# nhcha6/embodied-object-detection

Measured on AMD Instinct MI355X. Metric: frames/sec (640x640, implicit_memory); frames/sec/GPU = value / n_gpus, higher is better.
Workload: dtype f32

## Files before the change

embodied_object_detection_amd/_lib.py:

```python
from __future__ import annotations

import ctypes as C
import os

HERE = os.path.dirname(os.path.abspath(__file__))
LIB_PATH = os.environ.get("EOD_LIB_PATH") or os.path.join(HERE, "libeod_hip.so")

c_f32p = C.c_void_p
c_i32p = C.c_void_p
c_void_p = C.c_void_p


class EodError(RuntimeError):
    pass


_ERR = {-1: "EOD_ERR_BAD_DIMS", -2: "EOD_ERR_ALIGN", -3: "EOD_ERR_LAUNCH", -4: "EOD_ERR_NULL", -5: "EOD_ERR_CAPACITY"}


MAX_BATCH = 8
MAX_LEVELS = 40
SEMMAP_SCORES = 0x10000
SEMMAP_LOCATE = 0x40000
SEMMAP_PEAKS = 0x80000
SEMMAP_K_SHIFT, SEMMAP_RADIUS_SHIFT, SEMMAP_Q_SHIFT = 12, 20, 24


class EodConvDesc(C.Structure):
    _fields_ = [
        ("x", C.c_void_p), ("w", C.c_void_p), ("bias", C.c_void_p), ("res", C.c_void_p), ("y", C.c_void_p),
        ("workspace", C.c_void_p), ("workspace_bytes", C.c_size_t), ("m_count", C.c_void_p), ("m_unit", C.c_int32),
        ("m_segments", C.c_int32),
        ("N", C.c_int32), ("H", C.c_int32), ("W", C.c_int32), ("Cin", C.c_int32), ("OH", C.c_int32), ("OW", C.c_int32),
        ("Cout", C.c_int32), ("KH", C.c_int32), ("KW", C.c_int32), ("stride", C.c_int32), ("pad", C.c_int32),
        ("Kpad", C.c_int32), ("relu", C.c_int32), ("res_mode", C.c_int32), ("in_relu", C.c_int32),
        ("out_mode", C.c_int32), ("tap4", C.c_int32), ("force_tile", C.c_int32), ("force_splitk", C.c_int32),
        ("out_scale", C.c_float), ("levels", C.c_int32), ("level_off", C.c_int32 * (MAX_LEVELS + 1)), ("level_h", C.c_int32 * MAX_LEVELS),
        ("level_w", C.c_int32 * MAX_LEVELS), ("fuse_w", C.c_void_p), ("out_units", C.c_void_p), ("fuse_b", C.c_float), ("w_split", C.c_void_p),
        ("plan_rows", C.c_int32), ("lds_reserve", C.c_int32), ("gn_partial", C.c_void_p), ("gn_groups", C.c_int32),
        ("y2", C.c_void_p), ("split_n", C.c_int32), ("prefetch2", C.c_int32), ("gate", C.c_void_p),
        ("w_half", C.c_void_p), ("math", C.c_int32),
    ]


class EodConvPlan(C.Structure):
    _fields_ = [(n, C.c_int32) for n in ("tile", "bm", "bn", "bk", "splitk", "cps", "nchunks", "wavek", "glds", "tiles_m", "tiles_n",
                                         "gn_fused")]


class EodBoxRefine(C.Structure):
    _fields_ = [("deltas", C.c_void_p), ("ld", C.c_int32), ("wx", C.c_float), ("wy", C.c_float), ("ww", C.c_float), ("wh", C.c_float),
                ("clip", C.c_int32), ("img_w", C.c_float), ("img_h", C.c_float), ("boxes_out", C.c_void_p)]


class EodCenterNetLossDesc(C.Structure):
    _fields_ = [
        ("head_out", C.c_void_p), ("head_stride", C.c_int32), ("P", C.c_int32), ("levels", C.c_int32), ("level_off", C.c_int32 * 9),
        ("level_scale", C.c_float * 8), ("agn_heatmap", C.c_void_p), ("reg_targets", C.c_void_p), ("pos_inds", C.c_void_p),
        ("n_pos", C.c_int32), ("hm_focal_alpha", C.c_float), ("hm_focal_beta", C.c_float), ("loss_gamma", C.c_float),
        ("sigmoid_clamp", C.c_float), ("ignore_high_fp", C.c_float), ("pos_weight", C.c_float), ("neg_weight", C.c_float),
        ("reg_weight", C.c_float), ("num_pos_avg", C.c_float), ("reg_norm", C.c_float), ("counts_local", C.c_void_p),
        ("counts_total", C.c_void_p), ("world_size", C.c_float), ("d_head_out", C.c_void_p),
        ("losses", C.c_void_p), ("workspace", C.c_void_p), ("workspace_bytes", C.c_size_t),
    ]


class EodCenterNetTargetDesc(C.Structure):
    _fields_ = [
        ("gt_boxes", C.c_void_p), ("n_boxes", C.c_int32), ("levels", C.c_int32), ("level_off", C.c_int32 * 9), ("level_w", C.c_int32 * 8),
        ("level_stride", C.c_int32 * 8), ("soi_lo", C.c_float * 8), ("soi_hi", C.c_float * 8), ("hm_min_overlap", C.c_double),
        ("min_radius", C.c_double), ("agn_heatmap", C.c_void_p), ("reg_targets", C.c_void_p), ("pos_inds", C.c_void_p),
        ("counts", C.c_void_p),
    ]


class EodProposalDesc(C.Structure):
    _fields_ = [
        ("head_out", C.c_void_p), ("head_stride", C.c_int32), ("levels", C.c_int32), ("level_off", C.c_int32 * 6),
        ("level_w", C.c_int32 * 5), ("level_stride", C.c_int32 * 5), ("level_scale", C.c_float * 5),
        ("score_thresh", C.c_float), ("pre_nms_topk", C.c_int32), ("post_nms_topk", C.c_int32), ("nms_thresh", C.c_float),
# ... 152 lines not shown
    "eod_place_masks_workspace_bytes": (C.c_size_t, [C.c_int, C.c_int]),
    "eod_place_masks": (C.c_int, [C.c_void_p] * 4 + [C.c_int] * 7 + [C.c_void_p, C.c_void_p, C.c_size_t, C.c_void_p]),
}

REGIONS_SIGNATURES = {
    "eod_map_regions_workspace_bytes": (C.c_size_t, [C.c_int] * 3),
    "eod_map_regions": (C.c_int, [C.c_void_p] + [C.c_int] * 3 + [C.c_float] + [C.c_int] * 3 + [C.c_void_p] * 3 + [C.c_size_t, C.c_void_p]),
}

INVENTORY_SIGNATURES = {
    "eod_map_inventory_workspace_bytes": (C.c_size_t, [C.c_int] * 4),
    "eod_map_inventory": (C.c_int, [C.c_void_p] * 3 + [C.c_int] * 4 + [C.c_float] + [C.c_int] * 3 + [C.c_void_p] * 3 + [C.c_size_t, C.c_void_p]),
}

DESCRIBE_SIGNATURES = {
    "eod_describe_pool": (C.c_int, [C.c_void_p] * 3 + [C.c_int] * 2 + [C.c_void_p] * 5),
    "eod_describe_classify": (C.c_int, [C.c_void_p] * 2 + [C.c_int] * 3 + [C.c_void_p] * 4),
}

RELATIONS_SIGNATURES = {
    "eod_map_relations": (C.c_int, [C.c_void_p] * 2 + [C.c_int] * 6 + [C.c_void_p] * 12),
}

ROUTE_SIGNATURES = {
    "eod_map_route_workspace_bytes": (C.c_size_t, [C.c_int] * 2),
    "eod_map_route": (C.c_int, [C.c_void_p] * 3 + [C.c_int] * 8 + [C.c_void_p] * 11 + [C.c_size_t, C.c_void_p]),
}

CLEARANCE_SIGNATURES = {
    "eod_map_clearance_workspace_bytes": (C.c_size_t, [C.c_int] * 2),
    "eod_map_clearance": (C.c_int, [C.c_void_p] * 3 + [C.c_int] * 6 + [C.c_void_p] * 13 + [C.c_size_t, C.c_void_p]),
}

_lib = None


def load():
    global _lib
    if _lib is not None:
        return _lib
    if not os.path.exists(LIB_PATH):
        raise EodError(
            f"{LIB_PATH} is missing: the HIP extension is not built. Run `python -m embodied_object_detection_amd.build` "
            "(hipcc --offload-arch=gfx950). There is no CPU fallback for the product path.")
    lib = C.CDLL(LIB_PATH)
    for name, (res, args) in {**SIGNATURES, **PLACE_SIGNATURES, **REGIONS_SIGNATURES, **INVENTORY_SIGNATURES,
                              **DESCRIBE_SIGNATURES, **RELATIONS_SIGNATURES, **ROUTE_SIGNATURES, **CLEARANCE_SIGNATURES}.items():
        fn = getattr(lib, name)
        fn.restype = res
        fn.argtypes = args
    _lib = lib
    return lib


def check(status: int, what: str):
    if status != 0:
        raise EodError(f"{what} failed: {_ERR.get(status, status)}")
```

embodied_object_detection_amd/build.py:

```python
from __future__ import annotations

import os
import subprocess
import sys

HERE = os.path.dirname(os.path.abspath(__file__))
CSRC = os.path.join(HERE, "csrc")
LIB = os.path.join(HERE, "libeod_hip.so")
SOURCES = ["conv_igemm.hip", "conv_fp32.hip", "conv_pointwise.hip", "conv_bf16x3.hip", "conv_f16.hip", "elementwise.hip", "roi_align.hip", "select.hip", "heads.hip", "memory.hip", "semmap.hip", "place.hip", "regions.hip", "inventory.hip", "memory_read.hip", "memory_backward.hip", "conv_wgrad.hip", "train_losses.hip", "describe.hip", "relations.hip", "route.hip", "clearance.hip"]
ARCH = "gfx950"


def _stale() -> bool:
    if not os.path.exists(LIB):
        return True
    t = os.path.getmtime(LIB)
    deps = [os.path.join(CSRC, f) for f in os.listdir(CSRC)] + [os.path.join(HERE, "..", "include", h) for h in ("eod_hip.h", "eod_place.h", "eod_regions.h", "eod_inventory.h", "eod_describe.h", "eod_relations.h", "eod_route.h", "eod_clearance.h")]
    return any(os.path.getmtime(d) > t for d in deps if os.path.exists(d))


def _usage_file(src: str) -> str:
    return os.path.join(HERE, "build", src.replace(".hip", ".usage.txt"))


def resource_usage() -> dict:
    import re
    out = {}
    for src in SOURCES:
        f = _usage_file(src)
        if not os.path.exists(f):
            continue
        cur = None
        for line in open(f):
            m = re.search(r"Function Name: (\S+)", line)
            if m:
                cur = out.setdefault(m.group(1), {})
                continue
            for key, pat in (("vgprs", r"\bVGPRs: (\d+)"), ("scratch", r"ScratchSize \[bytes/lane\]: (\d+)"),
                             ("occupancy", r"Occupancy \[waves/SIMD\]: (\d+)"), ("lds", r"LDS Size \[bytes/block\]: (\d+)")):
                m = re.search(pat, line)
                if m and cur is not None:
                    cur[key] = int(m.group(1))
    return out


def scratch_offenders(usage: dict = None) -> list:
    usage = resource_usage() if usage is None else usage
    return sorted(k for k, v in usage.items() if v.get("scratch", 0) > 0)


# ... 50 lines not shown
```

embodied_object_detection_amd/csrc/conv_common.h:

```cpp
#pragma once
#include "eod_common.h"
#include "conv_border_order.h"
#include "../../include/eod_hip.h"

namespace eodconv {


struct ConvArgs {
  const float* x;
  const float* w;
  const float* bias;
  const float* res;
  const float* gate;
  float* y;
  float* partial;
  const int* m_count;
  int m_unit;
  int m_segs, seg_rows;
  const float* fuse_w;
  const int* out_units;
  float fuse_b;
  int N, H, W, Cin, OH, OW, Cout, KH, KW, stride, pad, Kpad;
  int M, nchunks, splitk, cps;
  int relu, res_mode, in_relu, out_mode;
  int tiles_m, tiles_n;
  float out_scale;
  int nlv;
  int lv_off[EOD_MAX_LEVELS + 1], lv_h[EOD_MAX_LEVELS], lv_w[EOD_MAX_LEVELS];
  unsigned x_bytes, w_bytes;
  const void* w3;
  unsigned w3_bytes;
  const void* wh;
  unsigned wh_bytes;
  double* gn_partial;
  int gn_groups;
  float* y2;
  int split_n;
  FastDiv div_ow, div_oh, div_cd, div_row;
  int border;
  FastDiv div_bh, div_bw, div_bi;
};

__device__ __forceinline__ int conv_row_limit(const ConvArgs& p, int M) {
  if (p.m_count && p.m_segs <= 1) {
    const int lim = *p.m_count * p.m_unit;
    M = lim < M ? lim : M;
  }
  return M;
}

__device__ __forceinline__ bool conv_row_active(const ConvArgs& p, int m) {
  if (!p.m_count || p.m_segs <= 1) return true;
  const int s = m / p.seg_rows;
  return m - s * p.seg_rows < p.m_count[s] * p.m_unit;
}

__device__ __forceinline__ bool conv_tile_active(const ConvArgs& p, int m0, int bm) {
  if (!p.m_count || p.m_segs <= 1) return true;
  const int last = (m0 + bm - 1 < p.M ? m0 + bm - 1 : p.M - 1);
  const int s0 = m0 / p.seg_rows, s1 = last / p.seg_rows;
  if (m0 - s0 * p.seg_rows < p.m_count[s0] * p.m_unit) return true;
  for (int s = s0 + 1; s <= s1; ++s)
    if (p.m_count[s] > 0) return true;
  return false;
}

__device__ __forceinline__ int border_rois(const ConvArgs& p) {
  const int c = *p.m_count;
  return c < p.N ? c : p.N;
}
__device__ __forceinline__ int border_storage_row(const ConvArgs& p, int m, int rois) {
  const BorderRow b = border_row(m, rois, p.OH, p.OW, p.div_ow, p.div_bh, p.div_bw, p.div_bi);
  return (b.img * p.OH + b.oy) * p.OW + b.ox;
// ... 98 lines not shown
```

embodied_object_detection_amd/csrc/conv_fp32.hip:

```cpp
#include "conv_operands.h"

namespace eodconv {
namespace {

template <int BM, int BN, int BK, bool TAP4, bool MULTI, int PIPE = 0>
__global__ __launch_bounds__(256) void conv_igemm_kernel(ConvArgs p) {
  constexpr bool BORDER = PIPE == 3;
  static_assert(!BORDER || (BM == 64 && BN == 64 && BK == 32 && !TAP4 && !MULTI), "border-major order: the plain 64x64 kernel");
  constexpr bool PF2 = PIPE == 1;
  constexpr bool DB = PIPE == 2;
  constexpr int LS = BK + 4;
  constexpr int TM = BM / 64, TN = BN / 64;
  constexpr int QPR = BK / 4;
  constexpr int RPP = 256 / QPR;
  constexpr int AR = BM / RPP, BR = BN / RPP;
  static_assert(!TAP4 || BK == 32, "the stem path stages one 7x7 tap per float4: BK must be 32");
  constexpr int BUF = (BM + BN) * LS;
  __shared__ __attribute__((aligned(16))) float lds[(DB ? 2 : 1) * BUF];
  float* As = lds;
  float* Bs = lds + BM * LS;

  const int tid = threadIdx.x;
  const int lane = tid & 63;
  const int wave = tid >> 6;
  const int wm = wave >> 1, wn = wave & 1;

  int M, tile_m, tile_n;
  if constexpr (BORDER) {
    if (!conv_claim_tile_border<BM>(p, M, tile_m, tile_n)) return;
  } else {
    const int t = conv_first_tile<BM>(p, M);
    if (t < 0) return;
    tile_m = t / p.tiles_n;
    tile_n = t - tile_m * p.tiles_n;
  }
  const int m0 = tile_m * BM, n0 = tile_n * BN;
  if (!conv_tile_active(p, m0, BM)) return;
  const int z = blockIdx.y;
  int c_end;
  const int c_begin = conv_chunk_range(p, p.cps, z, c_end);

  const int lr = tid / QPR, lq = tid % QPR;
  int a_off[AR], a_iy[AR], a_ix[AR];
  unsigned a_voff[AR];
  unsigned long long a_mask[AR];
  unsigned a_pitch[MULTI ? AR : 1];
  const int rois = BORDER ? border_rois(p) : 0;
#pragma unroll
  for (int i = 0; i < AR; ++i) {
    const int m = m0 + lr + RPP * i;
    const bool rowok = m < M;
    RowOrigin o;
    if constexpr (BORDER) o = conv_row_origin_border(p, m, rowok, rois);
    else o = conv_row_origin<MULTI>(p, m, rowok);
    a_iy[i] = rowok ? o.iy0 : -(1 << 28);
    a_ix[i] = o.ix0;
    a_off[i] = o.off;
    if (!TAP4) conv_row_address<MULTI>(p, o, rowok, lq, a_voff[i], a_mask[i], a_pitch[MULTI ? i : 0]);
  }
  unsigned w_voff[BR];
#pragma unroll
  for (int j = 0; j < BR; ++j) w_voff[j] = conv_w_row_offset(p, n0 + lr + RPP * j, lq);
  const __amdgpu_buffer_rsrc_t rsrc_x = conv_buffer(p.x, p.x_bytes);
  const __amdgpu_buffer_rsrc_t rsrc_w = conv_buffer(p.w, p.w_bytes);

  unsigned live = 0;
  if constexpr (BORDER) {
// ... 182 lines not shown
      if (tid < BM) {
        const int wr = tid >> 5, rr = tid & 31;
        const float v = red[(wr * 2 + 0) * 32 + rr] + red[(wr * 2 + 1) * 32 + rr] + p.fuse_b;
        const int m = m0 + tid;
        if (m < M) {
          const int tq = (int)fdiv((unsigned)m, p.div_ow);
          const int ox = m - tq * p.OW;
          const int img = (int)fdiv((unsigned)tq, p.div_oh);
          const int oy = tq - img * p.OH;
          const int unit = p.out_units ? p.out_units[img] : img;
          const int dy = tile_n >> 1, dx = tile_n & 1;
          p.y[((size_t)unit * 2 * p.OH + 2 * oy + dy) * (2 * p.OW) + 2 * ox + dx] = eod_sigmoid_precise(v);
        }
      }
      return;
    }
  }
  store_wave_tiles<TM, TN, BM == 64 && BN == 64, BORDER>(p, acc, m0 + wm * TM * 32, n0 + wn * TN * 32, M, z, lane);
}


template <int NW, bool MULTI>
__global__ __launch_bounds__(NW * 64) void conv_wavek_kernel(ConvArgs p) {
  constexpr int BK = 32;
  constexpr int LS = BK + 4;
  constexpr int AR = 4;
  __shared__ __attribute__((aligned(16))) float lds[NW * 2 * 32 * LS];
  const int tid = threadIdx.x;
  const int lane = tid & 63;
  const int wave = tid >> 6;
  float* As = lds + wave * (2 * 32 * LS);
  float* Bs = As + 32 * LS;

  int M;
  const int t = conv_first_tile<32>(p, M);
  if (t < 0) return;
  const int tile_m = t / p.tiles_n;
  const int tile_n = t - tile_m * p.tiles_n;
  const int m0 = tile_m * 32, n0 = tile_n * 32;
  if (!conv_tile_active(p, m0, 32)) return;

  int c_end;
  const int c_begin = conv_chunk_range(p, (p.nchunks + NW - 1) / NW, wave, c_end);

  const int lr = lane >> 3, lq = lane & 7;
  unsigned a_voff[AR];
  unsigned long long a_mask[AR];
  unsigned a_pitch[MULTI ? AR : 1];
  unsigned w_voff[AR];
#pragma unroll
  for (int i = 0; i < AR; ++i) {
    conv_row_address<MULTI>(p, m0 + lr + 8 * i, M, lq, a_voff[i], a_mask[i], a_pitch[MULTI ? i : 0]);
    w_voff[i] = conv_w_row_offset(p, n0 + lr + 8 * i, lq);
  }
  const __amdgpu_buffer_rsrc_t rsrc_x = conv_buffer(p.x, p.x_bytes);
  const __amdgpu_buffer_rsrc_t rsrc_w = conv_buffer(p.w, p.w_bytes);

  f32x4 ar0[AR], br0[AR], ar1[AR], br1[AR];
  ChunkWalker<BK, MULTI> walk(p, c_begin);
  auto load_chunk = [&](int chunk, f32x4 (&ar)[AR], f32x4 (&br)[AR]) {
    const int k0 = chunk * BK;
    const TapInfo ti = walk.next(p);
#pragma unroll
    for (int i = 0; i < AR; ++i) ar[i] = conv_load_a<MULTI>(rsrc_x, ti, a_voff[i], a_mask[i], a_pitch[MULTI ? i : 0]);
    if (p.in_relu) {
#pragma unroll
      for (int i = 0; i < AR; ++i) ar[i] = conv_relu4(ar[i]);
    }
#pragma unroll
    for (int j = 0; j < AR; ++j)
      br[j] = __builtin_bit_cast(f32x4, __builtin_amdgcn_raw_buffer_load_b128(rsrc_w, w_voff[j], k0 * 4, 0));
// ... 112 lines not shown
```

embodied_object_detection_amd/csrc/conv_igemm.hip:

```cpp
#include "conv_common.h"
#include "../../include/eod_hip.h"
#include <atomic>
#include <cstdlib>
#include <cstring>

namespace {

using namespace eodconv;

template <int VEC>
__global__ __launch_bounds__(256) void conv_splitk_reduce_kernel(ConvArgs p) {
  EOD_CHAIN_PRIO();
  const int M = conv_row_limit(p, p.M);
  const unsigned per_row = (unsigned)p.Cout / VEC;
  const unsigned total = (unsigned)M * per_row;
  const size_t slab = (size_t)p.M * p.Cout;
  for (unsigned idx = blockIdx.x * blockDim.x + threadIdx.x; idx < total; idx += gridDim.x * blockDim.x) {
    const unsigned m = fdiv(idx, p.div_row);
    if (!conv_row_active(p, (int)m)) continue;
    const unsigned n = (idx - m * per_row) * VEC;
    const float* src = p.partial + (size_t)m * p.Cout + n;
    if (VEC == 4) {
      f32x4 v = {0.f, 0.f, 0.f, 0.f};
      for (int zb = 0; zb < p.splitk; zb += 4) {
        f32x4 t[4];
#pragma unroll
        for (int j = 0; j < 4; ++j)
          if (zb + j < p.splitk) t[j] = *reinterpret_cast<const f32x4*>(src + (size_t)(zb + j) * slab);
#pragma unroll
        for (int j = 0; j < 4; ++j)
          if (zb + j < p.splitk) v += t[j];
      }
      epilogue_store<true>(p, v.x, (int)m, (int)n);
      epilogue_store<true>(p, v.y, (int)m, (int)n + 1);
// ... 57 lines not shown
    red[sub][col / cpg4][0] = s;
    red[sub][col / cpg4][1] = q;
  }
  __syncthreads();
  if ((int)threadIdx.x < p.gn_groups) {
    double ts = 0.0, tq = 0.0;
    for (int u = 0; u < nsub; ++u) {
      ts += red[u][threadIdx.x][0];
      tq += red[u][threadIdx.x][1];
    }
    p.gn_partial[((size_t)blockIdx.x * p.gn_groups + threadIdx.x) * 2 + 0] = ts;
    p.gn_partial[((size_t)blockIdx.x * p.gn_groups + threadIdx.x) * 2 + 1] = tq;
  }
}

std::atomic<int>& math_mode() {
  static std::atomic<int> v([] {
    const char* e = getenv("EOD_CONV_MATH");
    if (e && strcmp(e, "bf16x3") == 0) return EOD_MATH_BF16X3;
    if (e && strcmp(e, "f16") == 0) return EOD_MATH_F16;
    return EOD_MATH_FP32;
  }());
  return v;
}

struct Plan {
  int tile;
  int bk;
  int glds;
  int bm, bn, tiles_m, tiles_n, splitk, cps, nchunks;
  int wavek;
  int pw_np;
  int border;
};

constexpr int kForcePointwise = 30;

int effective_math(const EodConvDesc* d) { return d->math > 0 ? d->math - 1 : math_mode().load(std::memory_order_relaxed); }

bool pointwise_eligible(const EodConvDesc* d) {
  return effective_math(d) == EOD_MATH_FP32 && d->KH == 1 && d->KW == 1 && d->stride == 1 && d->pad == 0 && d->levels <= 0 && !d->tap4 &&
         d->Cin == d->Kpad && (d->Cin == 64 || d->Cin == 128 || d->Cin == 256) && d->Cout % 64 == 0 && d->out_mode == 0 &&
         (d->res_mode == 0 || d->res_mode == 1) && !d->in_relu && !d->gate && !d->m_count && d->split_n == 0 && !d->gn_partial &&
         d->lds_reserve == 0;
}

constexpr int kForceBorder = 43;
constexpr bool kBorderAuto = true;

bool border_eligible(const EodConvDesc* d) {
  return effective_math(d) == EOD_MATH_FP32 && d->KH == 3 && d->KW == 3 && d->stride == 1 && d->pad == 1 && d->levels <= 0 && !d->tap4 &&
         d->m_count && d->m_segments <= 1 && d->m_unit == d->OH * d->OW && d->OH >= 3 && d->OW >= 3 && d->Cin % 32 == 0 &&
         d->out_mode == 0 && d->res_mode == 0 && !d->in_relu && !d->gate && d->split_n == 0 && !d->gn_partial && d->prefetch2 == 0;
}

Plan make_plan(const EodConvDesc* d, int M) {
  static const int cfg[5][2] = {{128, 128}, {128, 64}, {64, 64}, {256, 128}, {64, 256}};
  Plan pl{};
  int pick = 2;
  const int ft = d->force_tile % 10, fbk = d->force_tile / 10;
  const bool half_ok = !d->tap4 && !d->in_relu;
  const bool f16_forced = (fbk == 8 || fbk == 9) && half_ok;
  if (f16_forced) pick = ft == 4 ? 3 : 2;
  else if (ft >= 1 && ft <= 3) pick = ft - 1;
  else if (ft == 4 && fbk == 5 && half_ok) pick = 3;
  const bool bk64_ok = !d->tap4 && d->Cin % 64 == 0 && d->Kpad % 64 == 0;
  pl.glds = f16_forced ? 3 : ((fbk == 5 && half_ok) ? 2 : 0);
// ... 67 lines not shown
  const bool pw_auto = d->force_tile == 0 && d->force_splitk == 0 && pointwise_eligible(d) && pl.splitk == 1 && !pl.wavek && tiles >= 256 &&
                       !(d->Kpad == 256 && d->Cout < 1024);
  if (pw_forced || pw_auto) {
    const int panels = d->Cout / 64;
    const long row_tiles = (Mp + 63) / 64;
    const long want = tiles >= 256 ? 512 : 1;
    int np = 1;
    for (int cand = 4; cand > 1; cand >>= 1)
      if (panels >= cand && row_tiles * ((panels + cand - 1) / cand) >= want) {
        np = cand;
        break;
      }
    pl.pw_np = np;
    pl.tile = 6;
    pl.glds = 0;
    pl.bk = 32;
    pl.nchunks = d->Kpad / 32;
    pl.bm = 64;
    pl.bn = 64 * np;
    pl.tiles_m = (M + 63) / 64;
    pl.tiles_n = (panels + np - 1) / np;
    pl.splitk = 1;
    pl.cps = pl.nchunks;
    pl.wavek = 0;
  }
  const bool border_forced = d->force_tile == kForceBorder && d->force_splitk <= 1;
  const bool border_auto = kBorderAuto && d->force_tile == 0 && border_eligible(d) && pl.glds == 0 && pl.tile == 3 && pl.bk == 32 &&
                           pl.splitk == 1 && !pl.wavek;
  if (border_forced) {
    pl.splitk = 1;
    pl.cps = pl.nchunks;
  }
  pl.border = (border_forced || border_auto) ? 1 : 0;
  return pl;
}

int total_rows(const EodConvDesc* d) { return d->levels > 0 ? d->level_off[d->levels] : d->N * d->OH * d->OW; }

int check_desc(const EodConvDesc* d) {
  if (!d || !d->x || !d->w || !d->y) return EOD_ERR_NULL;
  if (d->N <= 0 || d->Cin <= 0 || d->Cout <= 0) return EOD_ERR_BAD_DIMS;
  if (d->levels <= 0 && (d->H <= 0 || d->W <= 0 || d->OH <= 0 || d->OW <= 0)) return EOD_ERR_BAD_DIMS;
  if (d->KH <= 0 || d->KW <= 0 || d->stride <= 0 || d->pad < 0) return EOD_ERR_BAD_DIMS;
  if (d->Kpad % 32 != 0 || d->Kpad < d->KH * d->KW * d->Cin) return EOD_ERR_BAD_DIMS;
  if (d->tap4) {
    if (d->Cin != 4) return EOD_ERR_BAD_DIMS;
  } else {
    if (d->Cin % 32 != 0 || d->Kpad != d->KH * d->KW * d->Cin) return EOD_ERR_BAD_DIMS;
  }
  if (d->levels > 0) {
    if (d->levels > EOD_MAX_LEVELS || d->N != 1 || d->stride != 1 || d->KH != d->KW || d->pad != d->KH / 2 || d->tap4 || d->out_mode != 0 ||
        d->res_mode == 2 || d->level_off[0] != 0)
      return EOD_ERR_BAD_DIMS;
    for (int l = 0; l < d->levels; ++l)
      if (d->level_h[l] <= 0 || d->level_w[l] <= 0 || d->level_off[l + 1] - d->level_off[l] != d->level_h[l] * d->level_w[l])
        return EOD_ERR_BAD_DIMS;
  } else {
    if (d->OH != (d->H + 2 * d->pad - d->KH) / d->stride + 1) return EOD_ERR_BAD_DIMS;
    if (d->OW != (d->W + 2 * d->pad - d->KW) / d->stride + 1) return EOD_ERR_BAD_DIMS;
  }
  if (d->levels <= 0 && (long)d->N * d->H * d->W * d->Cin >= (1L << 29)) return EOD_ERR_BAD_DIMS;
  if ((long)d->Cout * d->Kpad >= (1L << 29)) return EOD_ERR_BAD_DIMS;
  if (d->KH * d->KW > 64) return EOD_ERR_BAD_DIMS;
  if ((long)total_rows(d) * (d->Cout > d->Cin ? d->Cout : d->Cin) >= (1L << 31)) return EOD_ERR_BAD_DIMS;
  if (d->out_mode == 1 && (d->Cout % 4 != 0)) return EOD_ERR_BAD_DIMS;
  if (d->out_mode == 2) {
// ... 17 lines not shown
  if (d->gate && (d->force_tile / 10 == 8 || d->force_tile / 10 == 9) &&
      (d->math != EOD_MATH_F16 + 1 || d->force_tile % 10 != 3 || d->levels > 0 || d->tap4 || d->in_relu))
    return EOD_ERR_BAD_DIMS;
  if (d->math < 0 || d->math > EOD_MATH_F16 + 1) return EOD_ERR_BAD_DIMS;
  if ((d->force_tile / 10 == 8 || d->force_tile / 10 == 9) && d->force_tile % 10 != 3 && d->force_tile % 10 != 4) return EOD_ERR_BAD_DIMS;
  if (d->lds_reserve < 0 || d->lds_reserve > 48 * 1024) return EOD_ERR_BAD_DIMS;
  if (d->force_tile == kForcePointwise && (!pointwise_eligible(d) || d->force_splitk > 1)) return EOD_ERR_BAD_DIMS;
  if (d->force_tile == kForceBorder && (!border_eligible(d) || d->force_splitk > 1)) return EOD_ERR_BAD_DIMS;
  if (d->split_n != 0) {
    if (!d->y2) return EOD_ERR_NULL;
    if (d->split_n < 0 || d->split_n >= d->Cout || d->out_mode != 0 || d->res_mode != 0 || d->levels > 0 || d->gn_partial)
      return EOD_ERR_BAD_DIMS;
  }
  if (d->gn_partial) {
    const int cpg = d->gn_groups > 0 ? d->Cout / d->gn_groups : 0;
    if (d->levels <= 0 || d->m_count || d->out_mode != 0 || d->gn_groups <= 0 || d->gn_groups > 64 || d->Cout % d->gn_groups != 0 ||
        cpg > 64 || (cpg & (cpg - 1)) != 0 || cpg < 4 || d->Cout % 4 != 0 || d->Cout > 1024 || 256 % (d->Cout / 4) != 0 ||
        64 % (cpg / 4) != 0)
      return EOD_ERR_BAD_DIMS;
  }
  if (!eod_aligned16(d->x) || !eod_aligned16(d->w) || !eod_aligned16(d->w_split) || !eod_aligned16(d->w_half)) return EOD_ERR_ALIGN;
  return EOD_OK;
}

}

extern "C" int eod_set_conv_math(int mode) {
  if (mode != EOD_MATH_FP32 && mode != EOD_MATH_BF16X3 && mode != EOD_MATH_F16) return EOD_ERR_BAD_DIMS;
  return math_mode().exchange(mode);
}

extern "C" int eod_get_conv_math(void) { return math_mode().load(); }

extern "C" size_t eod_conv_split_weights_bytes(int Cout, int Kpad) {
  return (Cout > 0 && Kpad > 0 && Kpad % 32 == 0) ? (size_t)Cout * Kpad * 6 : 0;
}

extern "C" int eod_conv_split_weights_bf16x3(const float* w, int Cout, int Kpad, void* out, eod_stream_t stream) {
  if (!w || !out) return EOD_ERR_NULL;
  if (Cout <= 0 || Kpad <= 0 || Kpad % 32 != 0 || (long)Cout * Kpad * 6 >= (1L << 32)) return EOD_ERR_BAD_DIMS;
  if (!eod_aligned16(w) || !eod_aligned16(out)) return EOD_ERR_ALIGN;
  launch_split_weights(w, out, Cout, Kpad, static_cast<hipStream_t>(stream));
  return eod_launch_status();
}

extern "C" size_t eod_conv_half_weights_bytes(int Cout, int Kpad) {
  return (Cout > 0 && Kpad > 0 && Kpad % 32 == 0) ? (size_t)Cout * Kpad * 2 : 0;
}

extern "C" int eod_conv_half_weights(const float* w, int Cout, int Kpad, void* out, eod_stream_t stream) {
  if (!w || !out) return EOD_ERR_NULL;
  if (Cout <= 0 || Kpad <= 0 || Kpad % 32 != 0 || (long)Cout * Kpad >= (1L << 29)) return EOD_ERR_BAD_DIMS;
  if (!eod_aligned16(w) || !eod_aligned16(out)) return EOD_ERR_ALIGN;
  launch_half_weights(w, out, Cout, Kpad, static_cast<hipStream_t>(stream));
  return eod_launch_status();
}

extern "C" int eod_conv2d_gn_fused(const EodConvDesc* d) {
  EodConvDesc t = *d;
  t.gn_partial = nullptr;
  if (check_desc(&t) != EOD_OK) return 0;
  return make_plan(&t, total_rows(&t)).splitk > 1 ? 1 : 0;
}

extern "C" int eod_conv2d_plan(const EodConvDesc* d, EodConvPlan* out) {
  if (!out) return EOD_ERR_NULL;
  const int st = check_desc(d);
  if (st != EOD_OK) return st;
  const Plan pl = make_plan(d, total_rows(d));
  out->tile = pl.tile; out->bm = pl.bm; out->bn = pl.bn; out->bk = pl.bk;
  out->splitk = pl.splitk; out->cps = pl.cps; out->nchunks = pl.nchunks;
  out->wavek = pl.wavek; out->glds = pl.glds;
  out->tiles_m = pl.tiles_m; out->tiles_n = pl.tiles_n;
  out->gn_fused = (d->gn_partial && pl.splitk > 1) ? 1 : 0;
  return EOD_OK;
}

extern "C" size_t eod_conv2d_workspace_bytes(const EodConvDesc* d) {
  if (check_desc(d) != EOD_OK) return 0;
  const int M = total_rows(d);
  const Plan pl = make_plan(d, M);
  if (pl.splitk <= 1) return 0;
  return (size_t)pl.splitk * M * d->Cout * sizeof(float);
}

extern "C" int eod_conv2d(const EodConvDesc* d, eod_stream_t stream) {
  const int st = check_desc(d);
  if (st != EOD_OK) return st;
  hipStream_t s = static_cast<hipStream_t>(stream);
  ConvArgs a{};
  a.x = d->x; a.w = d->w; a.bias = d->bias; a.res = d->res; a.y = d->y;
  a.partial = d->workspace;
  a.m_count = d->m_count; a.m_unit = d->m_unit;
  a.m_segs = d->m_segments > 1 ? d->m_segments : 1;
  a.seg_rows = a.m_segs > 1 ? (d->N / d->m_segments) * d->OH * d->OW : 0;
  a.fuse_w = d->fuse_w; a.out_units = d->out_units; a.fuse_b = d->fuse_b;
  a.N = d->N; a.H = d->H; a.W = d->W; a.Cin = d->Cin; a.OH = d->OH; a.OW = d->OW; a.Cout = d->Cout;
  a.KH = d->KH; a.KW = d->KW; a.stride = d->stride; a.pad = d->pad; a.Kpad = d->Kpad;
  a.M = total_rows(d);
  a.div_ow = eod_make_fastdiv((unsigned)(d->OW > 0 ? d->OW : 1));
  a.div_oh = eod_make_fastdiv((unsigned)(d->OH > 0 ? d->OH : 1));
  a.div_row = eod_make_fastdiv((unsigned)(d->Cout % 4 == 0 ? d->Cout / 4 : d->Cout));
  a.div_cd = eod_make_fastdiv((unsigned)((d->Cout >> 2) > 0 ? (d->Cout >> 2) : 1));
  a.div_bh = eod_make_fastdiv((unsigned)(d->OH > 2 ? d->OH - 2 : 1));
  a.div_bw = eod_make_fastdiv((unsigned)(d->OW > 2 ? d->OW - 2 : 1));
  a.div_bi = eod_make_fastdiv((unsigned)(d->OH > 2 && d->OW > 2 ? (d->OH - 2) * (d->OW - 2) : 1));
  {
    const size_t xe = d->levels > 0 ? (size_t)d->level_off[d->levels] * d->Cin : (size_t)d->N * d->H * d->W * d->Cin;
    a.x_bytes = (unsigned)(xe * sizeof(float));
    a.w_bytes = (unsigned)((size_t)d->Cout * d->Kpad * sizeof(float));
    a.w3 = d->w_split;
    a.w3_bytes = (unsigned)((size_t)d->Cout * d->Kpad * 6);
    a.wh = d->w_half;
    a.wh_bytes = (unsigned)((size_t)d->Cout * d->Kpad * 2);
  }
  a.nlv = d->levels > 0 ? d->levels : 0;
  for (int l = 0; l < a.nlv; ++l) {
    a.lv_off[l] = d->level_off[l];
    a.lv_h[l] = d->level_h[l];
    a.lv_w[l] = d->level_w[l];
  }
  if (a.nlv) a.lv_off[a.nlv] = d->level_off[a.nlv];
  a.relu = d->relu; a.res_mode = d->res_mode; a.in_relu = d->in_relu; a.out_mode = d->out_mode;
  a.gate = d->gate;
  a.out_scale = d->out_scale;
  a.gn_partial = d->gn_partial;
  a.gn_groups = d->gn_groups;
  a.y2 = d->y2;
  a.split_n = d->split_n;
  const Plan pl = make_plan(d, a.M);
  if (d->gn_partial && pl.splitk <= 1) return EOD_ERR_BAD_DIMS;
  a.nchunks = pl.nchunks;
  a.splitk = pl.splitk; a.cps = pl.cps; a.tiles_m = pl.tiles_m; a.tiles_n = pl.tiles_n;
  a.border = pl.border;
  if (pl.splitk > 1) {
    const size_t need = (size_t)pl.splitk * a.M * a.Cout * sizeof(float);
    if (!d->workspace || d->workspace_bytes < need) return EOD_ERR_CAPACITY;
  }
  dim3 grid(pl.tiles_m * pl.tiles_n, pl.splitk);
  if (pl.border) grid.x = (pl.tiles_m + 7) / 8 * 8 * pl.tiles_n;
  if (pl.pw_np) launch_conv_pointwise(a, pl.pw_np, grid, s);
  else if (pl.wavek) launch_conv_wavek(a, pl.wavek, grid, s);
  else if (pl.glds == 3) launch_conv_f16(a, pl.tile, pl.bk, grid, s);
  else if (pl.glds == 2) launch_conv_bf16x3(a, pl.tile, grid, s);
  else launch_conv_fp32(a, pl.tile, pl.bk, d->tap4 != 0, grid, s, d->lds_reserve, d->prefetch2);
  if (pl.splitk > 1) {
    const size_t total = (size_t)a.M * a.Cout;
    const bool vec = a.Cout % 4 == 0;
    int blocks = (int)((total / (vec ? 4 : 1) + 255) / 256);
    if (blocks > 2048) blocks = 2048;
    if (blocks < 1) blocks = 1;
    if (a.gn_partial) {
      int chunks = 0;
      for (int l = 0; l < a.nlv; ++l) chunks += (a.lv_off[l + 1] - a.lv_off[l] + EOD_GN_ROWS - 1) / EOD_GN_ROWS;
      hipLaunchKernelGGL(conv_splitk_reduce_gn_kernel, dim3(chunks), dim3(256), 0, s, a);
    } else if (vec) hipLaunchKernelGGL(conv_splitk_reduce_kernel<4>, dim3(blocks), dim3(256), 0, s, a);
    else hipLaunchKernelGGL(conv_splitk_reduce_kernel<1>, dim3(blocks), dim3(256), 0, s, a);
  }
  return eod_launch_status();
}
```

embodied_object_detection_amd/csrc/conv_operands.h:

```cpp
#pragma once
#include "conv_common.h"

namespace eodconv {

template <int BM>
__device__ __forceinline__ int conv_first_tile(const ConvArgs& p, int& M) {
  M = conv_row_limit(p, p.M);
  const int ntiles = ((M + BM - 1) / BM) * p.tiles_n;
  if ((int)blockIdx.x >= ntiles) return -1;
  return xcd_remap(blockIdx.x, ntiles);
}

template <int BM>
__device__ __forceinline__ bool conv_claim_tile_border(const ConvArgs& p, int& M, int& tile_m, int& tile_n) {
  M = conv_row_limit(p, p.M);
  const int live = (M + BM - 1) / BM;
  const int xcd = blockIdx.x & 7, k = blockIdx.x >> 3;
  const int g = k / p.tiles_n;
  const int r = g * 8 + xcd;
  tile_n = k - g * p.tiles_n;
  tile_m = live - 1 - r;
  return r < live;
}

__device__ __forceinline__ int conv_chunk_range(const ConvArgs& p, int per, int idx, int& c_end) {
  const int c_begin = idx * per;
  c_end = c_begin + per;
  if (c_end > p.nchunks) c_end = p.nchunks;
  return c_begin;
}

struct RowOrigin {
  int iy0, ix0, off, hh, ww;
};
template <bool MULTI>
__device__ __forceinline__ RowOrigin conv_row_origin(const ConvArgs& p, int m, bool rowok) {
  RowOrigin o = {0, 0, 0, 1, 1};
  if (rowok) {
    if (MULTI) {
      int l = 0;
      while (l + 1 < p.nlv && m >= p.lv_off[l + 1]) ++l;
      const int local = m - p.lv_off[l];
      o.ww = p.lv_w[l];
// ... 117 lines not shown
```

embodied_object_detection_amd/csrc/conv_pointwise.hip:

```cpp
#include "conv_operands.h"

namespace eodconv {
namespace {

template <int K>
struct PointwiseCfg {
  static constexpr int BKW = K == 256 ? 16 : 32;
  static constexpr int LSA = K + 4;
  static constexpr int LSW = BKW + 4;
  static constexpr int A_FLOATS = 64 * LSA;
  static constexpr int W_FLOATS = 64 * LSW;
  static constexpr int LDS_BYTES = (A_FLOATS + 2 * W_FLOATS) * 4;
  static constexpr int WG_PER_CU = K == 256 ? 2 : 3;
};

template <int K>
__global__ __launch_bounds__(256) __attribute__((amdgpu_waves_per_eu(PointwiseCfg<K>::WG_PER_CU))) void conv_pointwise_kernel(ConvArgs p, int np) {
  using Cfg = PointwiseCfg<K>;
  constexpr int BKW = Cfg::BKW, LSA = Cfg::LSA, LSW = Cfg::LSW;
  constexpr int NC = K / BKW;
  constexpr int KS = BKW / 8;
  constexpr int QPR = BKW / 4;
  constexpr int RPP = 256 / QPR;
  constexpr int BR = 64 / RPP;
  constexpr int AQ = K / 4;
  constexpr int AR = K / 16;
  static_assert(NC % 2 == 0, "stage parity");
  extern __shared__ __attribute__((aligned(16))) float lds[];
  float* As = lds;
  float* Ws = lds + Cfg::A_FLOATS;

  const int tid = threadIdx.x;
  const int lane = tid & 63;
  const int wave = tid >> 6;
  const int wm = wave >> 1, wn = wave & 1;

  int M;
  const int t = conv_first_tile<64>(p, M);
  if (t < 0) return;
  const int tile_m = t / p.tiles_n;
  const int grp = t - tile_m * p.tiles_n;
  const int m0 = tile_m * 64;
  const int panels = p.Cout >> 6;
  const int p0 = grp * np;
  const int p1 = p0 + np < panels ? p0 + np : panels;

  const __amdgpu_buffer_rsrc_t rsrc_x = conv_buffer(p.x, p.x_bytes);
  const __amdgpu_buffer_rsrc_t rsrc_w = conv_buffer(p.w, p.w_bytes);

  const int lr = tid / QPR, lq = tid % QPR;
  auto load_w = [&](int panel, int c, f32x4 (&wr)[BR]) {
    if (c >= NC) {
      c -= NC;
      ++panel;
    }
    if (panel >= p1) return;
#pragma unroll
    for (int j = 0; j < BR; ++j)
      wr[j] = __builtin_bit_cast(f32x4, __builtin_amdgcn_raw_buffer_load_b128(rsrc_w, conv_w_row_offset(p, panel * 64 + lr + RPP * j, lq),
                                                                              c * BKW * 4, 0));
  };
  auto store_w = [&](int buf, const f32x4 (&wr)[BR]) {
#pragma unroll
    for (int j = 0; j < BR; ++j) *reinterpret_cast<f32x4*>(Ws + buf * Cfg::W_FLOATS + (lr + RPP * j) * LSW + 4 * lq) = wr[j];
  };

  const int half = lane >> 5;
  const int m_base = m0 + wm * 32 + 4 * half;
  const int n_lane = wn * 32 + (lane & 31);
  auto load_res = [&](int panel, float (&rr)[16], float& bb) {
    const int n = panel * 64 + n_lane;
    if (p.bias) bb = p.bias[n];
    if (p.res_mode == 1) {
#pragma unroll
// ... 115 lines not shown
```

embodied_object_detection_amd/ops.py:

```python
from __future__ import annotations

import ctypes as C
from typing import Dict, Optional, Sequence, Tuple

import numpy as np
import torch

from . import _lib
from ._lib import EodConvDesc, EodDetDesc, EodMemWriteDesc, EodProposalDesc, check


_raw_stream = getattr(torch._C, "_cuda_getCurrentRawStream", None)


def _stream() -> int:
    if _raw_stream is not None:
        return _raw_stream(torch.cuda.current_device())
    return torch.cuda.current_stream().cuda_stream


def _ptr(t: Optional[torch.Tensor]) -> Optional[int]:
    return None if t is None else t.data_ptr()


# ... 8 lines not shown
    def __init__(self):
        self.bufs = {}

    def get(self, nbytes: int, device) -> torch.Tensor:
        key = (device.index if isinstance(device, torch.device) else str(device), _stream())
        buf = self.bufs.get(key)
        if buf is None or buf.numel() < nbytes:
            buf = torch.empty(max(int(nbytes), 1 << 20), dtype=torch.uint8, device=device)
            self.bufs[key] = buf
        return buf


_conv_ws = Workspace()


_CONV_MATH = {"fp32": 0, "bf16x3": 1, "f16": 2}
WGRAD_F16 = 512


def set_conv_math(mode: str) -> str:
    if mode not in _CONV_MATH:
        hint = ""
        if str(mode).lower() == "fp16":
            hint = (' ("fp16" / FP16 is the config key of autocast training: modeling.training.build_trainer / AmpTrainer, which choose '
                    'the arithmetic per launch; the process-wide inference arithmetic is "f16")')
        raise ValueError(f"conv math must be one of {sorted(_CONV_MATH)}, got {mode!r}{hint}")
    prev = _lib.load().eod_set_conv_math(_CONV_MATH[mode])
    check(min(prev, 0), "eod_set_conv_math")
    return {v: k for k, v in _CONV_MATH.items()}[prev]


def get_conv_math() -> str:
    return {v: k for k, v in _CONV_MATH.items()}[_lib.load().eod_get_conv_math()]


def fold_bn(w: torch.Tensor, bn_w, bn_b, bn_mean, bn_var, eps: float = 1e-5):
    scale = bn_w / torch.sqrt(bn_var + eps)
    return w * scale.view(-1, 1, 1, 1), bn_b - bn_mean * scale


def pack_conv_weight(w_oihw: torch.Tensor, cin_pad: Optional[int] = None) -> Tuple[torch.Tensor, int]:
    O, I, KH, KW = w_oihw.shape
    w = w_oihw.permute(0, 2, 3, 1).contiguous()
    if cin_pad is not None and cin_pad != I:
        wp = torch.zeros((O, KH, KW, cin_pad), dtype=w.dtype)
        wp[..., :I] = w
        w = wp
    K = w.shape[1] * w.shape[2] * w.shape[3]
    Kpad = (K + 31) // 32 * 32
    out = torch.zeros((O, Kpad), dtype=torch.float32)
    out[:, :K] = w.reshape(O, K)
    return out.contiguous(), Kpad


class Conv:

    def __init__(self, w_oihw: torch.Tensor, bias: Optional[torch.Tensor], stride: int = 1, pad: int = 0,
                 device="cuda", cin_pad: Optional[int] = None, deconv: bool = False, name: str = ""):
        self.name = name
        if deconv:
            Cin, Cout, kh, kw = w_oihw.shape
            assert kh == 2 and kw == 2
            w = w_oihw.permute(2, 3, 1, 0).reshape(4 * Cout, Cin, 1, 1).contiguous()
            self.out_mode = 1
            self.KH = self.KW = 1
            self.stride, self.pad = 1, 0
# ... 1644 lines not shown
```

include/eod_hip.h:

```cpp
#ifndef EOD_HIP_H
#define EOD_HIP_H
#include <stddef.h>
#include <stdint.h>

#ifdef __cplusplus
extern "C" {
#endif

typedef void* eod_stream_t;

#define EOD_OK 0
#define EOD_ERR_BAD_DIMS (-1)
#define EOD_ERR_ALIGN (-2)
#define EOD_ERR_LAUNCH (-3)
#define EOD_ERR_NULL (-4)
#define EOD_ERR_CAPACITY (-5)

#define EOD_MAX_BATCH 8
#define EOD_MAX_LEVELS 40

int eod_abi_version(void);

typedef struct EodConvDesc {
  const float* x;
// ... 15 lines not shown
  int32_t force_tile;
  int32_t force_splitk;
  float out_scale;
  int32_t levels;
  int32_t level_off[EOD_MAX_LEVELS + 1];
  int32_t level_h[EOD_MAX_LEVELS];
  int32_t level_w[EOD_MAX_LEVELS];
  const float* fuse_w;
  const int32_t* out_units;
  float fuse_b;
  const void* w_split;
  int32_t plan_rows;
  int32_t lds_reserve;
  double* gn_partial;
  int32_t gn_groups;
  float* y2;
  int32_t split_n;
  int32_t prefetch2;
  const float* gate;
  const void* w_half;
  int32_t math;
} EodConvDesc;
int eod_conv2d(const EodConvDesc* d, eod_stream_t stream);
int eod_conv2d_gn_fused(const EodConvDesc* d);
size_t eod_conv2d_workspace_bytes(const EodConvDesc* d);
typedef struct EodConvPlan {
  int32_t tile;
  int32_t bm, bn, bk;
  int32_t splitk, cps, nchunks;
  int32_t wavek;
  int32_t glds;
  int32_t tiles_m, tiles_n;
  int32_t gn_fused;
} EodConvPlan;
int eod_conv2d_plan(const EodConvDesc* d, EodConvPlan* out);
#define EOD_MATH_FP32 0
#define EOD_MATH_BF16X3 1
#define EOD_MATH_F16 2
int eod_set_conv_math(int mode);
int eod_get_conv_math(void);
size_t eod_conv_split_weights_bytes(int Cout, int Kpad);
int eod_conv_split_weights_bf16x3(const float* w, int Cout, int Kpad, void* out, eod_stream_t stream);
size_t eod_conv_half_weights_bytes(int Cout, int Kpad);
int eod_conv_half_weights(const float* w, int Cout, int Kpad, void* out, eod_stream_t stream);

int eod_preprocess_image(const uint8_t* img_chw, float* out_nhwc4, int H, int W, int Hp, int Wp,
                         const float* mean3, const float* std3, eod_stream_t stream);
int eod_maxpool3x3s2(const float* x, float* y, int N, int H, int W, int C, int OH, int OW, eod_stream_t stream);
size_t eod_groupnorm_workspace_bytes(const int32_t* level_off_host, int levels, int groups);
int eod_groupnorm_relu(const float* x, float* y, const float* gamma, const float* beta, const int32_t* level_off_host,
                       int levels, int C, int groups, float eps, float* stats, int partial_ready, eod_stream_t stream);
size_t eod_groupnorm_partial_offset(int levels, int groups);
size_t eod_groupnorm_backward_workspace_bytes(const int32_t* level_off_host, int levels, int C);
int eod_groupnorm_relu_backward(const float* x, const float* y, const float* dy, const float* gamma, const int32_t* level_off_host,
                                int levels, int C, int groups, float eps, const float* fwd_stats, void* workspace, float* dx,
                                float* dgamma, float* dbeta, eod_stream_t stream);
int eod_mask_predictor_sigmoid(const float* x, const float* w, float bias, float* prob, int rows, int C,
                               const int32_t* unit_count, int unit_rows, const int32_t* out_units ,
                               eod_stream_t stream);

typedef struct EodBoxRefine {
  const float* deltas;
  int32_t ld;
  float wx, wy, ww, wh;
  int32_t clip;
  float img_w, img_h;
// ... 294 lines not shown
```

Baseline: 322.9.

## Choose row- or column-major conv tile order per layer from an L2 fetch model

Adds a per-launch tile rasterization order for the implicit-GEMM conv kernels. A host-side model estimates how many A (activation) and B (weight) tile bytes each XCD's contiguous range of tiles would fetch under row-major versus column-major order, then picks the cheaper one. In auto mode this applies only to wavek==4 plans without glds, border or out_mode 2. The goal is less redundant operand traffic through each XCD's L2. Kernels now go through a shared conv_claim_tile helper, and the EodConvPlan struct gains a field, which changes the ABI.

Result: no change. 320.1 (-0.9%).

```diff
diff --git a/embodied_object_detection_amd/_lib.py b/embodied_object_detection_amd/_lib.py
--- a/embodied_object_detection_amd/_lib.py
+++ b/embodied_object_detection_amd/_lib.py
@@ -45,7 +45,7 @@
 
 class EodConvPlan(C.Structure):
     _fields_ = [(n, C.c_int32) for n in ("tile", "bm", "bn", "bk", "splitk", "cps", "nchunks", "wavek", "glds", "tiles_m", "tiles_n",
-                                         "gn_fused")]
+                                         "gn_fused", "order")]
 
 
 class EodBoxRefine(C.Structure):
@@ -264,6 +264,11 @@
     "eod_map_clearance": (C.c_int, [C.c_void_p] * 3 + [C.c_int] * 6 + [C.c_void_p] * 13 + [C.c_size_t, C.c_void_p]),
 }
 
+CONV_ORDER_SIGNATURES = {
+    "eod_set_conv_tile_order": (C.c_int, [C.c_int]),
+    "eod_get_conv_tile_order": (C.c_int, []),
+}
+
 _lib = None
 
 
@@ -277,7 +282,8 @@
             "(hipcc --offload-arch=gfx950). There is no CPU fallback for the product path.")
     lib = C.CDLL(LIB_PATH)
     for name, (res, args) in {**SIGNATURES, **PLACE_SIGNATURES, **REGIONS_SIGNATURES, **INVENTORY_SIGNATURES,
-                              **DESCRIBE_SIGNATURES, **RELATIONS_SIGNATURES, **ROUTE_SIGNATURES, **CLEARANCE_SIGNATURES}.items():
+                              **DESCRIBE_SIGNATURES, **RELATIONS_SIGNATURES, **ROUTE_SIGNATURES, **CLEARANCE_SIGNATURES,
+                              **CONV_ORDER_SIGNATURES}.items():
         fn = getattr(lib, name)
         fn.restype = res
         fn.argtypes = args
diff --git a/embodied_object_detection_amd/build.py b/embodied_object_detection_amd/build.py
--- a/embodied_object_detection_amd/build.py
+++ b/embodied_object_detection_amd/build.py
@@ -15,7 +15,7 @@
     if not os.path.exists(LIB):
         return True
     t = os.path.getmtime(LIB)
-    deps = [os.path.join(CSRC, f) for f in os.listdir(CSRC)] + [os.path.join(HERE, "..", "include", h) for h in ("eod_hip.h", "eod_place.h", "eod_regions.h", "eod_inventory.h", "eod_describe.h", "eod_relations.h", "eod_route.h", "eod_clearance.h")]
+    deps = [os.path.join(CSRC, f) for f in os.listdir(CSRC)] + [os.path.join(HERE, "..", "include", h) for h in ("eod_hip.h", "eod_place.h", "eod_regions.h", "eod_inventory.h", "eod_describe.h", "eod_relations.h", "eod_route.h", "eod_clearance.h", "eod_conv_order.h")]
     return any(os.path.getmtime(d) > t for d in deps if os.path.exists(d))
 
 
diff --git a/embodied_object_detection_amd/csrc/conv_common.h b/embodied_object_detection_amd/csrc/conv_common.h
--- a/embodied_object_detection_amd/csrc/conv_common.h
+++ b/embodied_object_detection_amd/csrc/conv_common.h
@@ -1,6 +1,7 @@
 #pragma once
 #include "eod_common.h"
 #include "conv_border_order.h"
+#include "conv_tile_order.h"
 #include "../../include/eod_hip.h"
 
 namespace eodconv {
@@ -39,6 +40,7 @@
   FastDiv div_ow, div_oh, div_cd, div_row;
   int border;
   FastDiv div_bh, div_bw, div_bi;
+  int order;
 };
 
 __device__ __forceinline__ int conv_row_limit(const ConvArgs& p, int M) {
diff --git a/embodied_object_detection_amd/csrc/conv_fp32.hip b/embodied_object_detection_amd/csrc/conv_fp32.hip
--- a/embodied_object_detection_amd/csrc/conv_fp32.hip
+++ b/embodied_object_detection_amd/csrc/conv_fp32.hip
@@ -29,10 +29,7 @@
   if constexpr (BORDER) {
     if (!conv_claim_tile_border<BM>(p, M, tile_m, tile_n)) return;
   } else {
-    const int t = conv_first_tile<BM>(p, M);
-    if (t < 0) return;
-    tile_m = t / p.tiles_n;
-    tile_n = t - tile_m * p.tiles_n;
+    if (!conv_claim_tile<BM>(p, M, tile_m, tile_n)) return;
   }
   const int m0 = tile_m * BM, n0 = tile_n * BN;
   if (!conv_tile_active(p, m0, BM)) return;
@@ -281,11 +278,8 @@
   float* As = lds + wave * (2 * 32 * LS);
   float* Bs = As + 32 * LS;
 
-  int M;
-  const int t = conv_first_tile<32>(p, M);
-  if (t < 0) return;
-  const int tile_m = t / p.tiles_n;
-  const int tile_n = t - tile_m * p.tiles_n;
+  int M, tile_m, tile_n;
+  if (!conv_claim_tile<32>(p, M, tile_m, tile_n)) return;
   const int m0 = tile_m * 32, n0 = tile_n * 32;
   if (!conv_tile_active(p, m0, 32)) return;
 
diff --git a/embodied_object_detection_amd/csrc/conv_igemm.hip b/embodied_object_detection_amd/csrc/conv_igemm.hip
--- a/embodied_object_detection_amd/csrc/conv_igemm.hip
+++ b/embodied_object_detection_amd/csrc/conv_igemm.hip
@@ -1,5 +1,6 @@
 #include "conv_common.h"
 #include "../../include/eod_hip.h"
+#include "../../include/eod_conv_order.h"
 #include <atomic>
 #include <cstdlib>
 #include <cstring>
@@ -123,7 +124,33 @@
   int wavek;
   int pw_np;
   int border;
+  int order;
 };
+
+std::atomic<int>& tile_order_mode() {
+  static std::atomic<int> v([] {
+    const char* e = getenv("EOD_CONV_TILE_ORDER");
+    if (e && strcmp(e, "row") == 0) return EOD_TILE_ORDER_ROW;
+    if (e && strcmp(e, "col") == 0) return EOD_TILE_ORDER_COL;
+    if (e && strcmp(e, "bytes") == 0) return EOD_TILE_ORDER_BYTES;
+    return EOD_TILE_ORDER_AUTO;
+  }());
+  return v;
+}
+
+int pick_tile_order(const EodConvDesc* d, const Plan& pl) {
+  const bool takes = pl.glds == 0 && !pl.border && d->out_mode != 2;
+  if (!takes) return kTileRowMajor;
+  const int mode = tile_order_mode().load(std::memory_order_relaxed);
+  if (mode == EOD_TILE_ORDER_ROW) return kTileRowMajor;
+  if (mode == EOD_TILE_ORDER_COL) return kTileColMajor;
+  if (mode == EOD_TILE_ORDER_AUTO && pl.wavek != 4) return kTileRowMajor;
+  const double in_rows = d->levels > 0 ? (double)d->level_off[d->levels] : (double)d->N * d->H * d->W;
+  const double a_tile = in_rows * d->Cin * 4.0 / pl.tiles_m;
+  const double b_tile = (double)d->Cout * d->Kpad * 4.0 / pl.tiles_n;
+  const TileFetch row = conv_tile_fetch(kTileRowMajor, pl.tiles_m, pl.tiles_n), col = conv_tile_fetch(kTileColMajor, pl.tiles_m, pl.tiles_n);
+  return a_tile * col.a + b_tile * col.b < a_tile * row.a + b_tile * row.b ? kTileColMajor : kTileRowMajor;
+}
 
 constexpr int kForcePointwise = 30;
 
@@ -257,6 +284,7 @@
     pl.cps = pl.nchunks;
   }
   pl.border = (border_forced || border_auto) ? 1 : 0;
+  pl.order = pick_tile_order(d, pl);
   return pl;
 }
 
@@ -340,6 +368,13 @@
 
 extern "C" int eod_get_conv_math(void) { return math_mode().load(); }
 
+extern "C" int eod_set_conv_tile_order(int mode) {
+  if (mode < EOD_TILE_ORDER_AUTO || mode > EOD_TILE_ORDER_BYTES) return EOD_ERR_BAD_DIMS;
+  return tile_order_mode().exchange(mode);
+}
+
+extern "C" int eod_get_conv_tile_order(void) { return tile_order_mode().load(); }
+
 extern "C" size_t eod_conv_split_weights_bytes(int Cout, int Kpad) {
   return (Cout > 0 && Kpad > 0 && Kpad % 32 == 0) ? (size_t)Cout * Kpad * 6 : 0;
 }
@@ -381,6 +416,7 @@
   out->wavek = pl.wavek; out->glds = pl.glds;
   out->tiles_m = pl.tiles_m; out->tiles_n = pl.tiles_n;
   out->gn_fused = (d->gn_partial && pl.splitk > 1) ? 1 : 0;
+  out->order = pl.order;
   return EOD_OK;
 }
 
@@ -441,6 +477,7 @@
   a.nchunks = pl.nchunks;
   a.splitk = pl.splitk; a.cps = pl.cps; a.tiles_m = pl.tiles_m; a.tiles_n = pl.tiles_n;
   a.border = pl.border;
+  a.order = pl.order;
   if (pl.splitk > 1) {
     const size_t need = (size_t)pl.splitk * a.M * a.Cout * sizeof(float);
     if (!d->workspace || d->workspace_bytes < need) return EOD_ERR_CAPACITY;
diff --git a/embodied_object_detection_amd/csrc/conv_operands.h b/embodied_object_detection_amd/csrc/conv_operands.h
--- a/embodied_object_detection_amd/csrc/conv_operands.h
+++ b/embodied_object_detection_amd/csrc/conv_operands.h
@@ -9,6 +9,12 @@
   const int ntiles = ((M + BM - 1) / BM) * p.tiles_n;
   if ((int)blockIdx.x >= ntiles) return -1;
   return xcd_remap(blockIdx.x, ntiles);
+}
+
+template <int BM>
+__device__ __forceinline__ bool conv_claim_tile(const ConvArgs& p, int& M, int& tile_m, int& tile_n) {
+  M = conv_row_limit(p, p.M);
+  return conv_tile_of(p.order, (int)blockIdx.x, (M + BM - 1) / BM, p.tiles_n, tile_m, tile_n);
 }
 
 template <int BM>
diff --git a/embodied_object_detection_amd/csrc/conv_pointwise.hip b/embodied_object_detection_amd/csrc/conv_pointwise.hip
--- a/embodied_object_detection_amd/csrc/conv_pointwise.hip
+++ b/embodied_object_detection_amd/csrc/conv_pointwise.hip
@@ -35,11 +35,8 @@
   const int wave = tid >> 6;
   const int wm = wave >> 1, wn = wave & 1;
 
-  int M;
-  const int t = conv_first_tile<64>(p, M);
-  if (t < 0) return;
-  const int tile_m = t / p.tiles_n;
-  const int grp = t - tile_m * p.tiles_n;
+  int M, tile_m, grp;
+  if (!conv_claim_tile<64>(p, M, tile_m, grp)) return;
   const int m0 = tile_m * 64;
   const int panels = p.Cout >> 6;
   const int p0 = grp * np;
diff --git a/embodied_object_detection_amd/csrc/conv_tile_order.h b/embodied_object_detection_amd/csrc/conv_tile_order.h
--- /dev/null
+++ b/embodied_object_detection_amd/csrc/conv_tile_order.h
@@ -0,0 +1,52 @@
+#pragma once
+
+#if defined(__HIPCC__)
+#define EOD_TILE_FN __host__ __device__ __forceinline__
+#else
+#define EOD_TILE_FN static inline
+#endif
+
+namespace eodconv {
+
+constexpr int kTileRowMajor = 0;
+constexpr int kTileColMajor = 1;
+
+EOD_TILE_FN int tile_xcd_range(int bid, int n) {
+  const int q = n >> 3, r = n & 7;
+  const int xcd = bid & 7, k = bid >> 3;
+  const int base = (xcd < r) ? xcd * (q + 1) : r * (q + 1) + (xcd - r) * q;
+  return base + k;
+}
+
+EOD_TILE_FN bool conv_tile_of(int order, int bid, int live_rows, int tiles_n, int& tile_m, int& tile_n) {
+  const int ntiles = live_rows * tiles_n;
+  if (bid >= ntiles) return false;
+  const int id = tile_xcd_range(bid, ntiles);
+  if (order == kTileColMajor) {
+    tile_n = id / live_rows;
+    tile_m = id - tile_n * live_rows;
+  } else {
+    tile_m = id / tiles_n;
+    tile_n = id - tile_m * tiles_n;
+  }
+  return true;
+}
+
+struct TileFetch {
+  long a, b;
+};
+static inline TileFetch conv_tile_fetch(int order, int rows, int cols) {
+  const int n = rows * cols;
+  const int inner = order == kTileColMajor ? rows : cols;
+  long outer_sum = 0, inner_sum = 0;
+  for (int x = 0; x < 8 && x < n; ++x) {
+    const int lo = tile_xcd_range(x, n);
+    const int len = n / 8 + (x < n % 8 ? 1 : 0);
+    const int hi = lo + len - 1;
+    outer_sum += hi / inner - lo / inner + 1;
+    inner_sum += len < inner ? len : inner;
+  }
+  return order == kTileColMajor ? TileFetch{inner_sum, outer_sum} : TileFetch{outer_sum, inner_sum};
+}
+
+}
diff --git a/embodied_object_detection_amd/ops.py b/embodied_object_detection_amd/ops.py
--- a/embodied_object_detection_amd/ops.py
+++ b/embodied_object_detection_amd/ops.py
@@ -64,6 +64,17 @@
 
 def get_conv_math() -> str:
     return {v: k for k, v in _CONV_MATH.items()}[_lib.load().eod_get_conv_math()]
+
+
+_TILE_ORDER = {"auto": 0, "row": 1, "col": 2, "bytes": 3}
+
+
+def set_conv_tile_order(mode: str) -> str:
+    if mode not in _TILE_ORDER:
+        raise ValueError(f"conv tile order must be one of {sorted(_TILE_ORDER)}, got {mode!r}")
+    prev = _lib.load().eod_set_conv_tile_order(_TILE_ORDER[mode])
+    check(min(prev, 0), "eod_set_conv_tile_order")
+    return {v: k for k, v in _TILE_ORDER.items()}[prev]
 
 
 def fold_bn(w: torch.Tensor, bn_w, bn_b, bn_mean, bn_var, eps: float = 1e-5):
diff --git a/include/eod_conv_order.h b/include/eod_conv_order.h
--- /dev/null
+++ b/include/eod_conv_order.h
@@ -0,0 +1,19 @@
+#ifndef EOD_CONV_ORDER_H
+#define EOD_CONV_ORDER_H
+#include "eod_hip.h"
+
+#ifdef __cplusplus
+extern "C" {
+#endif
+
+#define EOD_TILE_ORDER_AUTO 0
+#define EOD_TILE_ORDER_ROW 1
+#define EOD_TILE_ORDER_COL 2
+#define EOD_TILE_ORDER_BYTES 3
+int eod_set_conv_tile_order(int mode);
+int eod_get_conv_tile_order(void);
+
+#ifdef __cplusplus
+}
+#endif
+#endif
diff --git a/include/eod_hip.h b/include/eod_hip.h
--- a/include/eod_hip.h
+++ b/include/eod_hip.h
@@ -71,6 +71,7 @@
   int32_t glds;
   int32_t tiles_m, tiles_n;
   int32_t gn_fused;
+  int32_t order;
 } EodConvPlan;
 int eod_conv2d_plan(const EodConvDesc* d, EodConvPlan* out);
 #define EOD_MATH_FP32 0
```
